# Rikorose/DeepFilterNet

Measured on NVIDIA H100. Metric: 48kHz audio-sec/sec (batched enhance), higher is better.
Workload: dtype f32 (bf16x3 tensor-core contractions, fp32 accumulate; DSP and gates IEEE fp32)

## Files before the change

### deepfilternet_b200/csrc/dfb_dwpw.cuh

```cuda
#pragma once
#include <cuda_runtime.h>
#include <stdint.h>

namespace dfb {

constexpr int kCh = 64;

__device__ __forceinline__ unsigned long long f2_pack(float lo, float hi) {
    unsigned long long r;
    asm("mov.b64 %0, {%1, %2};" : "=l"(r) : "f"(lo), "f"(hi));
    return r;
}
__device__ __forceinline__ void f2_unpack(unsigned long long v, float &lo, float &hi) {
    asm("mov.b64 {%0, %1}, %2;" : "=f"(lo), "=f"(hi) : "l"(v));
}
__device__ __forceinline__ unsigned long long f2_fma(unsigned long long a, unsigned long long b, unsigned long long c) {
    float a0, a1, b0, b1, c0, c1;
    f2_unpack(a, a0, a1);
    f2_unpack(b, b0, b1);
    f2_unpack(c, c0, c1);
    return f2_pack(fmaf(a0, b0, c0), fmaf(a1, b1, c1));
}

enum DwMode { DW_S1 = 0, DW_S2 = 1, DW_T2 = 2 };
constexpr int kLdA = kCh + 4;

struct DwPwParams {
    const float *in;
    const float *path;
    const float *ps, *pb;
    const float *dw;
    const float *pw;
    const float *bias;
    float *out;
    unsigned short *out_hi, *out_lo;
    int64_t in_fs, path_fs, out_fs;
    int T, Fin, Fout, kt, NF, lookahead;
    int fo_magic;
    const float *mk_e0;
    const float *mk_ps, *mk_pb;
    const float *mk_w;
    const float *mk_bias;
    float *mk_out;
    const int64_t *first;
    int64_t w0;
};


struct DwTaps {
    float4 wd[9];
    float4 ps4, pb4;
};

__device__ __forceinline__ void dw_load_taps(const DwPwParams &p, int cq, DwTaps &tp) {
#pragma unroll
    for (int i = 0; i < 9; i++) tp.wd[i] = make_float4(0.f, 0.f, 0.f, 0.f);
#pragma unroll
    for (int i = 0; i < 9; i++)
        if (i >= (3 - p.kt) * 3) tp.wd[i] = *reinterpret_cast<const float4 *>(p.dw + (i - (3 - p.kt) * 3) * kCh + cq * 4);
    tp.ps4 = make_float4(0.f, 0.f, 0.f, 0.f);
    tp.pb4 = tp.ps4;
    if (p.path) {
        tp.ps4 = *reinterpret_cast<const float4 *>(p.ps + cq * 4);
        tp.pb4 = *reinterpret_cast<const float4 *>(p.pb + cq * 4);
    }
}

template <int MODE>
__device__ __forceinline__ float4 dw_prologue(const DwPwParams &p, const DwTaps &tp, int b, int t, int fo, int cq) {
    float4 acc = make_float4(0.f, 0.f, 0.f, 0.f);
#pragma unroll
    for (int dt = 0; dt < 3; dt++) {
        if (dt < 3 - p.kt) continue;
        const int tq = t - (2 - dt) + p.lookahead;
        if (tq < 0 || tq >= p.T) continue;
#pragma unroll
        for (int df = 0; df < 3; df++) {
            int fi;
            float4 wv;
            if (MODE == DW_S1) { fi = fo + df - 1; wv = tp.wd[dt * 3 + df]; }
            else if (MODE == DW_S2) { fi = 2 * fo + df - 1; wv = tp.wd[dt * 3 + df]; }
            else {
                if (df == 2) continue;
                if ((fo & 1) == 0) { if (df == 1) continue; fi = fo >> 1; wv = tp.wd[dt * 3 + 1]; }
                else if (df == 0) { fi = fo >> 1; wv = tp.wd[dt * 3 + 2]; }
                else { fi = (fo >> 1) + 1; wv = tp.wd[dt * 3 + 0]; }
            }
            if (fi < 0 || fi >= p.Fin) continue;
            const int64_t o = ((int64_t)b * p.T + tq);
            float4 x = *reinterpret_cast<const float4 *>(p.in + o * p.in_fs + fi * kCh + cq * 4);
            if (p.path) {
                float4 e = *reinterpret_cast<const float4 *>(p.path + o * p.path_fs + fi * kCh + cq * 4);
                x.x += fmaxf(e.x * tp.ps4.x + tp.pb4.x, 0.f);
                x.y += fmaxf(e.y * tp.ps4.y + tp.pb4.y, 0.f);
                x.z += fmaxf(e.z * tp.ps4.z + tp.pb4.z, 0.f);
                x.w += fmaxf(e.w * tp.ps4.w + tp.pb4.w, 0.f);
            }
            acc.x += x.x * wv.x; acc.y += x.y * wv.y; acc.z += x.z * wv.z; acc.w += x.w * wv.w;
        }
// ... 6 lines not shown
```

### deepfilternet_b200/csrc/dfb_model.cu

```cuda
#include <cuda_bf16.h>

#include <algorithm>
#include <cmath>
#include <cstring>
#include <functional>
#include <map>
#include <numeric>
#include <string>

#include "dfb_common.cuh"
#include "dfb_dwpw.cuh"
#include "dfb_ptx.cuh"

namespace dfb {


enum Act { ACT_NONE = 0, ACT_RELU = 1, ACT_TANH = 2, ACT_SIGMOID = 3 };

__device__ __forceinline__ float act_apply(float x, int act) {
    switch (act) {
        case ACT_RELU: return fmaxf(x, 0.f);
        case ACT_TANH: return tanhf(x);
        case ACT_SIGMOID: return 1.f / (1.f + expf(-x));
        default: return x;
    }
}
__device__ __forceinline__ float sigmoidf_(float x) { return 1.f / (1.f + expf(-x)); }

constexpr int kInFrames = 8;
template <int CIN>
__global__ void __launch_bounds__(256)
k_conv_in(const float *__restrict__ x, const float *__restrict__ w , const float *__restrict__ bias,
          float *__restrict__ out, int T, int F, int kt, int lookahead, int Tsx ,
          int Tx ,
          int tp_min ,
          const RaggedRow *__restrict__ rg , int64_t w0 ,
          const int64_t *__restrict__ first ) {
    extern __shared__ float s_in[];
    const int b = blockIdx.y, t0 = blockIdx.x * kInFrames;
    const int rows = kInFrames + kt - 1, ld = (F + 2) * CIN;
    if (rg) Tx = min(Tx, (int)(rg[b].Tf - w0));
    if (first) tp_min = max(tp_min, stream_first(first, b, w0));
    for (int i = threadIdx.x; i < rows * ld; i += blockDim.x) {
        int r = i / ld, j = i - r * ld;
        int f = j / CIN - 1, ci = j - (f + 1) * CIN;
        int tp = t0 - (kt - 1) + r;
        float v = 0.f;
        if (f >= 0 && f < F && tp >= tp_min && tp + lookahead < Tx) v = x[(((int64_t)b * Tsx + tp + lookahead) * F + f) * CIN + ci];
        s_in[i] = v;
    }
    const int cq = threadIdx.x & 15, fl = threadIdx.x >> 4;
    unsigned long long wr[9 * CIN][2];
#pragma unroll
    for (int i = 0; i < 9 * CIN; i++) {
        const float4 v = (i >= (3 - kt) * 3 * CIN) ? *reinterpret_cast<const float4 *>(w + (i - (3 - kt) * 3 * CIN) * kCh + cq * 4)
                                                   : make_float4(0.f, 0.f, 0.f, 0.f);
        wr[i][0] = f2_pack(v.x, v.y); wr[i][1] = f2_pack(v.z, v.w);
    }
    const float4 bv = *reinterpret_cast<const float4 *>(bias + cq * 4);
    const unsigned long long b01 = f2_pack(bv.x, bv.y), b23 = f2_pack(bv.z, bv.w);
    __syncthreads();
    for (int fr = 0; fr < kInFrames; fr++) {
        int t = t0 + fr;
        if (t >= T) break;
        for (int f = fl; f < F; f += 16) {
            unsigned long long a01 = b01, a23 = b23;
#pragma unroll
            for (int dt = 0; dt < 3; dt++) {
                if (dt < 3 - kt) continue;
                const float *row = s_in + (fr + dt - (3 - kt)) * ld + f * CIN;
#pragma unroll
                for (int j = 0; j < 3 * CIN; j++) {
                    const float xv = row[j];
                    const unsigned long long xx = f2_pack(xv, xv);
                    a01 = f2_fma(xx, wr[dt * 3 * CIN + j][0], a01);
                    a23 = f2_fma(xx, wr[dt * 3 * CIN + j][1], a23);
                }
            }
            float4 acc;
            f2_unpack(a01, acc.x, acc.y); f2_unpack(a23, acc.z, acc.w);
            acc.x = fmaxf(acc.x, 0.f); acc.y = fmaxf(acc.y, 0.f); acc.z = fmaxf(acc.z, 0.f); acc.w = fmaxf(acc.w, 0.f);
            *reinterpret_cast<float4 *>(out + (((int64_t)b * T + t) * F + f) * kCh + cq * 4) = acc;
        }
    }
}

template <int MODE>
__global__ void __launch_bounds__(256) k_dwpw(DwPwParams p) {
    extern __shared__ __align__(16) float smem[];
    float *Ws = smem;
    float *As = smem + kCh * kCh;
    const int b = blockIdx.y, t0 = blockIdx.x * p.NF;
    const int tid = threadIdx.x;
    const int nf = min(p.NF, p.T - t0);
    const int R = nf * p.Fout;
// ... 587 lines not shown
extern "C" int64_t dfb_model_workspace_bytes(const dfb_model *m) { return m ? (int64_t)m->arena.cap : 0; }

namespace {

int run_gl(cudaStream_t s, const float *x, int64_t ldx, const float *w, const float *bias, const float *res,
           int64_t ldr, float *y, int64_t ldy, int64_t M, int G, int I, int Hh, int act, float oscale = 1.f,
           float ooffset = 0.f, unsigned short *y_hi = nullptr, unsigned short *y_lo = nullptr) {
    GlParams p{x, ldx, w, bias, res, ldr, y, ldy, M, G, I / G, Hh / G, act, oscale, ooffset, y_hi, y_lo};
    if ((p.Ig % 4) || (ldx % 4)) return fail(DFB_ERR_UNSUPPORTED, "grouped linear: K not a multiple of 4");
    if (G > 1 && (p.Hg % 4)) return fail(DFB_ERR_UNSUPPORTED, "grouped linear: group width %d not a multiple of 4", p.Hg);
    int tiles = (p.Hg + kGlBN - 1) / kGlBN;
    int gpc = (p.Hg < kGlBN && kGlBN % p.Hg == 0) ? (kGlBN / p.Hg < G ? kGlBN / p.Hg : G) : 1;
    dim3 grid((unsigned)((M + kGlBM - 1) / kGlBM), (unsigned)(((G + gpc - 1) / gpc) * tiles));
    static const bool detail = getenv("DFB_PROF_DETAIL") && atoi(getenv("DFB_PROF_DETAIL"));
    char name[64];
    if (detail) snprintf(name, sizeof name, "k_grouped_linear[%dx%d/%d]", I, Hh, G);
    else snprintf(name, sizeof name, "%s", p.G == 1 && p.bias && p.Hg >= 512 ? "k_grouped_linear[gru_proj]" : "k_grouped_linear");
    DFB_PROF(name, s);
    k_grouped_linear<<<grid, 256, 0, s>>>(p);
    DFB_LAUNCH_CHECK();
    return DFB_OK;
}

int run_gru(dfb_model *m, cudaStream_t s, const GruLayer *lw, int layers, int H, const float *res_last, float *y,
            float *xproj, int B, int T, const unsigned short *x_hi, const unsigned short *x_lo,
            unsigned short *pl_hi, unsigned short *pl_lo, int wide, unsigned short *out_hi, unsigned short *out_lo,
            bool *out_planes_ok, const GruChunk *ck) {
    if (out_planes_ok) *out_planes_ok = false;
    if (!x_hi || !x_lo || !pl_hi || !pl_lo) return fail(DFB_ERR_INVALID, "GRU: input planes and scratch planes are required");
    const int t0 = ck ? ck->t0 : 0, Tn = T - t0;
    const int64_t M = (int64_t)B * T;
    const unsigned short *cur_hi = x_hi, *cur_lo = x_lo;
    for (int l = 0; l < layers; l++) {
        const GruLayer &g = lw[l];
        int rc;
        if ((rc = launch_gemm_bf16x3(s, cur_hi, cur_lo, H, g.w_ih_hi, g.w_ih_lo, g.b_ih, xproj, 3 * H, M, 3 * H, H))) return rc;
        const bool last = l == layers - 1;
        float *dst = last ? y : nullptr;
        float *hs = ck && ck->h ? ck->h + (int64_t)l * ck->Bs * H : nullptr;
        GruWindow gw{ck && ck->have_state ? hs : nullptr, hs, t0, T, ck ? ck->first : nullptr, ck ? ck->w0 : 0};
        unsigned short *hi = last ? out_hi : pl_hi, *lo = last ? out_lo : pl_lo;
        if ((rc = launch_gru_tc(s, xproj, g.w_hh, g.b_hh, last ? res_last : nullptr, dst, hi, lo, B, Tn,
                                Tn <= m->gru_dbg_steps ? m->gru_dbg : nullptr, wide, last ? 1 : 0, &gw, H)))
            return rc;
        if (last && hi && out_planes_ok) *out_planes_ok = true;
        cur_hi = pl_hi; cur_lo = pl_lo;
    }
    return DFB_OK;
}

}
namespace dfb {
template <int MODE>
int launch_dwpw_tc(cudaStream_t s, DwPwParams p, const float *w_sw, int B);
}
namespace {

template <int MODE>
int run_dwpw(cudaStream_t s, DwPwParams p, int B, const float *w_sw = nullptr) {
    if (w_sw) return launch_dwpw_tc<MODE>(s, p, w_sw, B);
    static PerDeviceOnce attr_once;
    const int smem = (kCh * kCh + 128 * kLdA) * 4;
    if (auto once_guard = attr_once.first()) {
        DFB_CUDA(cudaFuncSetAttribute(k_dwpw<MODE>, cudaFuncAttributeMaxDynamicSharedMemorySize, smem));
    }
    p.NF = 128 / p.Fout;
    if (p.NF < 1) p.NF = 1;
    if (p.NF * p.Fout > 128 || (p.NF * p.Fout) % 4) return fail(DFB_ERR_UNSUPPORTED, "dwpw tile: Fout = %d", p.Fout);
    dim3 grid((unsigned)((p.T + p.NF - 1) / p.NF), (unsigned)B);
    DFB_PROF("k_dwpw", s);
    k_dwpw<MODE><<<grid, 256, smem, s>>>(p);
    DFB_LAUNCH_CHECK();
    return DFB_OK;
}

}

struct FwdBufs {
    float *e0, *e1, *e2, *e3, *c0, *c1, *emb_in, *emb, *g_a, *g_b, *xproj, *dec_emb, *d3, *d2, *d1, *dfc;
    unsigned short *ga_hi, *ga_lo, *gh_hi, *gh_lo;
    float *g_a2, *xproj2, *dfskip;
    unsigned short *ga2_hi, *ga2_lo, *gh2_hi, *gh2_lo;
    unsigned short *c1_hi, *c1_lo, *embin_hi, *embin_lo, *gb_hi, *gb_lo, *emb_hi, *emb_lo, *dfc_hi, *dfc_lo;
};

struct FwdBufsV1 {
    float *e0, *e1, *e2, *e3, *c0, *c1, *c1g, *cemb, *emb, *xproj, *xproj2, *y[3], *embo, *dec_old, *dec, *p3, *p2, *p1, *p0, *d3, *d2, *d1,
        *z[2], *dfc;
    unsigned short *emb_hi, *emb_lo, *y_hi[3], *y_lo[3], *embo_hi, *embo_lo, *z_hi[2], *z_lo[2], *dfc_hi, *dfc_lo, *scr_hi, *scr_lo;
};
static size_t fwd_plan_v1(const dfb_model_config &c, size_t M, Arena *a, FwdBufsV1 *f) {
    const int E = c.nb_erb, Fd = c.nb_df, H = c.emb_hidden;
    size_t bytes = 0;
    auto take = [&](size_t n) -> float * {
        bytes += (n * 4 + 255) & ~size_t(255);
        return a ? a->take<float>(n) : nullptr;
    };
    auto take16 = [&](size_t n) { return reinterpret_cast<unsigned short *>(take((n + 1) / 2)); };
    FwdBufsV1 t{};
    t.e0 = take(M * E * kCh); t.e1 = take(M * (E / 2) * kCh); t.e2 = take(M * (E / 4) * kCh); t.e3 = take(M * (E / 4) * kCh);
    t.c0 = take(M * Fd * kCh); t.c1 = take(M * (Fd / 2) * kCh); t.c1g = take(M * (Fd / 2) * kCh);
    t.cemb = take(M * H); t.emb = take(M * H); t.xproj = take(M * 3 * H); t.xproj2 = take(M * 3 * H);
    for (int i = 0; i < 3; i++) { t.y[i] = take(M * H); t.y_hi[i] = take16(M * H); t.y_lo[i] = take16(M * H); }
    for (int i = 0; i < 2; i++) { t.z[i] = take(M * H); t.z_hi[i] = take16(M * H); t.z_lo[i] = take16(M * H); }
    t.embo = take(M * H); t.dec_old = take(M * H); t.dec = take(M * H); t.dfc = take(M * H);
    t.p3 = take(M * (E / 4) * kCh); t.p2 = take(M * (E / 4) * kCh); t.p1 = take(M * (E / 2) * kCh); t.p0 = take(M * E * kCh);
    t.d3 = take(M * (E / 4) * kCh); t.d2 = take(M * (E / 2) * kCh); t.d1 = take(M * E * kCh);
    t.emb_hi = take16(M * H); t.emb_lo = take16(M * H); t.embo_hi = take16(M * H); t.embo_lo = take16(M * H);
    t.dfc_hi = take16(M * H); t.dfc_lo = take16(M * H); t.scr_hi = take16(M * H); t.scr_lo = take16(M * H);
    if (f) *f = t;
    return bytes + 4096;
}

// ... 128 lines not shown
    m->dbg["emb"] = {f.emb, M * emb_dim}; m->dbg["dec_emb"] = {f.dec_emb, M * ED}; m->dbg["d3"] = {f.d3, M * ED};
    m->dbg["d2"] = {f.d2, M * (E / 2) * kCh}; m->dbg["d1"] = {f.d1, M * E * kCh}; m->dbg["dfc"] = {f.dfc, M * Hd};
    m->dbg["g_a"] = {f.g_a, M * (H > Hd ? H : Hd)}; m->dbg["g_b"] = {f.g_b, M * (H > Hd ? H : Hd)};
    m->dbg["xproj"] = {f.xproj, M * 3 * (H > Hd ? H : Hd)};
    m->dbg["emb_in_hi"] = {reinterpret_cast<const float *>(f.embin_hi), M * emb_in_dim / 2};
    m->dbg["emb_in_lo"] = {reinterpret_cast<const float *>(f.embin_lo), M * emb_in_dim / 2};
    m->dbg["dfc_hi"] = {reinterpret_cast<const float *>(f.dfc_hi), M * Hd / 2};
    m->dbg["dfc_lo"] = {reinterpret_cast<const float *>(f.dfc_lo), M * Hd / 2};
    const int64_t e3_fs = c.enc_concat ? 2 * ED : ED;
    const bool keep_ga = c.model_kind == 2;
    float *const enc_ga = w.enc_in.bx ? nullptr : f.g_a;
    float *const erb_ga = !keep_ga && w.erb_in.bx ? nullptr : f.g_a;
    float *const df_ga = !keep_ga && w.df_in.bx ? nullptr : f.g_a2;
    float *const enc_gb = w.enc_out.bx ? nullptr : f.g_b;
    float *const erb_gb = w.erb_out.bx ? nullptr : f.g_b;
    float *const dfc = c.model_kind != 2 && w.df_out.bx ? nullptr : f.dfc;
    if (!erb_ga) m->dbg.erase("g_a");
    if (!erb_gb) m->dbg.erase("g_b");
    if (!dfc) m->dbg.erase("dfc");
    struct Pl { unsigned short *hi, *lo; int64_t ld; bool ok; };
    Pl pl_c1{f.c1_hi, f.c1_lo, (int64_t)Fd / 2 * kCh, false}, pl_embin{f.embin_hi, f.embin_lo, emb_in_dim, false},
       pl_gb{f.gb_hi, f.gb_lo, H, false}, pl_emb{f.emb_hi, f.emb_lo, emb_dim, false}, pl_dfc{f.dfc_hi, f.dfc_lo, Hd, false},
       pl_ga{f.ga_hi, f.ga_lo, H, false}, pl_ga2{f.ga2_hi, f.ga2_lo, Hd, false};
    auto ensure_planes = [&](cudaStream_t st, const float *x, int64_t ldx, int K, Pl &pl) -> int {
        if (pl.ok) return DFB_OK;
        if (pl.ld != K) return fail(DFB_ERR_INVALID, "plane pitch mismatch");
        if (!x) return fail(DFB_ERR_INVALID, "planes requested of an activation whose fp32 form was not written");
        int r = launch_to_planes(st, x, ldx, M, K, pl.hi, pl.lo);
        if (!r) pl.ok = true;
        return r;
    };
    auto gl = [&](cudaStream_t st, const Gl &g, const float *x, int64_t ldx, Pl *xin, int act,
                  const float *res, int64_t ldr, float *y, int64_t ldy, Pl *yout, int64_t ycol = 0) -> int {
        int r;
        unsigned short *yh = yout ? yout->hi + ycol : nullptr, *yl = yout ? yout->lo + ycol : nullptr;
        if (xin && g.bx) {
            if ((r = ensure_planes(st, x, ldx, g.I, *xin))) return r;
            r = launch_gl_bx(st, xin->hi, xin->lo, xin->ld, g.img, res, ldr, y, ldy, yh, yl, yout ? yout->ld : 0, M, g.G, g.I / g.G,
                             g.H / g.G, act, 1.f, 0.f);
            if (r != DFB_ERR_UNSUPPORTED) {
                if (!r && yout) yout->ok = true;
                return r;
            }
        }
        if (!x || !y)
            return fail(DFB_ERR_UNSUPPORTED, "grouped linear %dx%d/%d: the tensor-core kernel cannot take this launch and the fp32 %s "
                        "the FFMA kernel needs is not written", g.I, g.H, g.G, x ? "output" : "input");
        const bool ffma_planes = yout && yout->ld == ldy;
        r = run_gl(st, x, ldx, g.w, nullptr, res, ldr, y, ldy, M, g.G, g.I, g.H, act, 1.f, 0.f, ffma_planes ? yh : nullptr, ffma_planes ? yl : nullptr);
        if (!r && yout) yout->ok = ffma_planes;
        return r;
    };

    {
        dim3 grid((unsigned)((T + kInFrames - 1) / kInFrames), (unsigned)B);
        int smem = (kInFrames + c.inp_kt - 1) * (E + 2) * 4;
        DFB_PROF("k_conv_in[erb_conv0]", s);
        k_conv_in<1><<<grid, 256, smem, s>>>(d_feat_erb, w.erb_conv0.w, w.erb_conv0.b, f.e0, T, E, c.inp_kt, c.conv_lookahead, Tsx, Tx, 0, rows, W0, first);
        DFB_LAUNCH_CHECK();
    }
    cudaStream_t sa = serial ? s : L.aux;
    DFB_CUDA(cudaEventRecord(L.ev_fork_enc, s));
    DFB_CUDA(cudaStreamWaitEvent(sa, L.ev_fork_enc, 0));
    auto mk = [&](const Blk &k, const float *in, int Fin, int64_t in_fs, float *out, int Fout, int64_t out_fs, int kt) {
        DwPwParams p{};
        p.in = in; p.Fin = Fin; p.in_fs = in_fs; p.out = out; p.Fout = Fout; p.out_fs = out_fs; p.kt = kt; p.T = T;
        p.lookahead = 0;
        p.first = first; p.w0 = W0; p.dw = k.dw; p.bias = k.b;
        return p;
    };
    {
        {
            dim3 grid((unsigned)((T + kInFrames - 1) / kInFrames), (unsigned)B);
            int smem = (kInFrames + c.inp_kt - 1) * (Fd + 2) * 2 * 4;
            DFB_PROF("k_conv_in[df_conv0]", sa);
            k_conv_in<2><<<grid, 256, smem, sa>>>(d_feat_spec, w.df_conv0.w, w.df_conv0.b, f.c0, T, Fd, c.inp_kt, c.conv_lookahead, Tsx, Tx, 0, rows, W0, first);
            DFB_LAUNCH_CHECK();
            DFB_CUDA(cudaEventRecord(L.ev_c0, sa));
        }
        if (w.fused_emb) m->dbg.erase("c1");
        if (!w.fused_emb) {
            DwPwParams p = mk(w.df_conv1, f.c0, Fd, (int64_t)Fd * kCh, f.c1, Fd / 2, (int64_t)Fd / 2 * kCh, c.conv_kt);
            p.out_hi = pl_c1.hi; p.out_lo = pl_c1.lo; pl_c1.ok = true;
            if ((rc = run_dwpw<DW_S2>(sa, p, B, w.df_conv1.pw_sw))) return rc;
        }
        DFB_CUDA(cudaEventRecord(L.ev_join_enc, sa));
        DFB_CUDA(cudaStreamWaitEvent(sl, L.ev_c0, 0));
        if (!df_convp_built(c.df_order, c.df_pathway_kt))
            return fail(DFB_ERR_UNSUPPORTED, "df_order %d / df_pathway_kernel_size_t %d (built kernels: df_order 5, kt 1-5)",
                        c.df_order, c.df_pathway_kt);
        if (Fd % 2) return fail(DFB_ERR_UNSUPPORTED, "df pathway conv: odd nb_df");
        if ((rc = launch_df_convp_tc(sl, f.c0, w.df_convp.w_sw, w.df_convp.w2, w.df_convp.b, d_coefs, B, T, Fd, c.df_order,
                                     c.df_pathway_kt, first, W0)))
            return rc;
        DFB_CUDA(cudaEventRecord(L.ev_convp, sl));
    }
    {
        DwPwParams p = mk(w.erb_conv1, f.e0, E, (int64_t)E * kCh, f.e1, E / 2, (int64_t)E / 2 * kCh, c.conv_kt);
        if ((rc = run_dwpw<DW_S2>(s, p, B, w.erb_conv1.pw_sw))) return rc;
        p = mk(w.erb_conv2, f.e1, E / 2, (int64_t)E / 2 * kCh, f.e2, E / 4, (int64_t)E / 4 * kCh, c.conv_kt);
        if ((rc = run_dwpw<DW_S2>(s, p, B, w.erb_conv2.pw_sw))) return rc;
        p = mk(w.erb_conv3, f.e2, E / 4, (int64_t)E / 4 * kCh, f.e3, E / 4, e3_fs, c.conv_kt);
        if (c.enc_concat) { p.out_hi = pl_embin.hi; p.out_lo = pl_embin.lo; }
        if ((rc = run_dwpw<DW_S1>(s, p, B, w.erb_conv3.pw_sw))) return rc;

    }
    DFB_CUDA(cudaStreamWaitEvent(s, L.ev_join_enc, 0));
    {
        const int I = Fd / 2 * kCh;
        if (w.fused_emb) {
            const int G = c.g_df_fc_emb;
            rc = launch_df_emb(s, f.c0, M, T, Fd, c.conv_kt, w.df_conv1.dw, w.df_conv1.b, w.df_conv1.pw_sw, w.df_fc_emb.img, G, I / G, ED / G,
                               c.enc_concat ? nullptr : f.e3, ED, pl_embin.hi + (c.enc_concat ? ED : 0), pl_embin.lo + (c.enc_concat ? ED : 0),
                               pl_embin.ld, first, W0);
            if (!rc) pl_embin.ok = true;
            m->dbg.erase("emb_in");
        } else if (c.enc_concat) {
            rc = gl(s, w.df_fc_emb, f.c1, I, &pl_c1, ACT_RELU, nullptr, 0, f.emb_in + ED, emb_in_dim, &pl_embin, ED);
        } else {
            rc = gl(s, w.df_fc_emb, f.c1, I, &pl_c1, ACT_RELU, f.e3, ED, f.emb_in, emb_in_dim, &pl_embin);
        }
        if (rc) return rc;
    }
    {
        if ((rc = gl(s, w.enc_in, w.fused_emb ? nullptr : f.emb_in, emb_in_dim, &pl_embin, ACT_RELU, nullptr, 0, enc_ga, H, &pl_ga)))
            return rc;
        float *gout = c.g_enc_out ? enc_gb : f.emb;
        Pl &pl_gout = c.g_enc_out ? pl_gb : pl_emb;
        if ((rc = run_gru(m, s, w.enc_gru.data(), c.enc_gru_layers, H, nullptr, gout, f.xproj, B, T, f.ga_hi, f.ga_lo,
                          f.gh_hi, f.gh_lo, 0, pl_gout.hi, pl_gout.lo, &pl_gout.ok, cx ? &ck_enc : nullptr))) return rc;
        if (c.g_enc_out) {
            if ((rc = gl(s, w.enc_out, enc_gb, H, &pl_gb, ACT_RELU, nullptr, 0, f.emb, emb_dim, &pl_emb))) return rc;
        }
        if ((rc = ensure_planes(s, f.emb, emb_dim, emb_dim, pl_emb))) return rc;
        if (d_lsnr && (rc = run_gl(s, f.emb, emb_dim, w.lsnr.w, w.lsnr.b, nullptr, 0, d_lsnr, 1, M, 1, emb_dim, 1, ACT_SIGMOID, c.lsnr_scale,
                                   c.lsnr_offset)))
            return rc;
    }
    DFB_CUDA(cudaEventRecord(L.ev_fork, s));
    if (!serial) { s = L.dhi; sa = L.daux; DFB_CUDA(cudaStreamWaitEvent(s, L.ev_fork, 0)); }
    DFB_CUDA(cudaStreamWaitEvent(sa, L.ev_fork, 0));
    if (cx && cx->wait_dec) {
        DFB_CUDA(cudaStreamWaitEvent(s, cx->wait_dec, 0));
        DFB_CUDA(cudaStreamWaitEvent(sa, cx->wait_dec, 0));
    }
    static const char *wide_env = getenv("DFB_WIDE_BRANCH");
    const int wide_df = !wide_env || !strcmp(wide_env, "df") || !strcmp(wide_env, "both");
    const int wide_erb = wide_env && (!strcmp(wide_env, "erb") || !strcmp(wide_env, "both"));
    const bool early_skip = c.g_df_skip && c.model_kind != 2;
    if (early_skip) {
        if ((rc = gl(s, w.df_skip, f.emb, emb_dim, &pl_emb, ACT_NONE, nullptr, 0, f.dfskip, Hd, nullptr))) return rc;
        DFB_CUDA(cudaEventRecord(L.ev_skip, s));
// ... 2272 lines not shown
```

### deepfilternet_b200/csrc/dfb_tc.cu

```cuda
#include <cooperative_groups.h>
#include <atomic>
#include <map>
#include <mutex>
#include <cuda.h>
#include <cuda_bf16.h>

#include "dfb_common.cuh"
#include "dfb_dwpw.cuh"
#include "dfb_ptx.cuh"

namespace dfb {

constexpr int kBxBM = 128, kBxBN = 128, kBxBK = 64, kBxStages = 3, kBxThreads = 288;
constexpr int kBxBox = 128 * 128;

struct BxSmem {
    alignas(1024) unsigned char x[kBxStages][2][kBxBox];
    alignas(1024) unsigned char w[kBxStages][2][kBxBox];
    alignas(8) uint64_t full[kBxStages];
    uint64_t empty[kBxStages];
};

__global__ void __launch_bounds__(kBxThreads, 1)
k_gemm_bf16x3(const __grid_constant__ CUtensorMap tmXhi, const __grid_constant__ CUtensorMap tmXlo,
// ... 9 lines not shown
        fence_barrier_init();
    }
    __syncthreads();
    if (warp == 8) {
        if (lane == 0) {
            tma_prefetch_desc(&tmXhi); tma_prefetch_desc(&tmXlo); tma_prefetch_desc(&tmWhi); tma_prefetch_desc(&tmWlo);
            for (int kb = 0; kb < nkb; kb++) {
                const int s = kb % kBxStages, n = kb / kBxStages;
                if (n > 0) mbar_wait(&sm.empty[s], (n - 1) & 1);
                mbar_expect_tx(&sm.full[s], 4 * kBxBox);
                tma_load_2d(sm.x[s][0], &tmXhi, kb * kBxBK, m0, &sm.full[s]);
                tma_load_2d(sm.x[s][1], &tmXlo, kb * kBxBK, m0, &sm.full[s]);
                tma_load_2d(sm.w[s][0], &tmWhi, kb * kBxBK, n0, &sm.full[s]);
                tma_load_2d(sm.w[s][1], &tmWlo, kb * kBxBK, n0, &sm.full[s]);
            }
        }
        return;
    }
    const int wm = (warp & 3) * 32, wn = (warp >> 2) * 64;
    float acc[2][8][4];
#pragma unroll
    for (int a = 0; a < 2; a++)
#pragma unroll
        for (int b = 0; b < 8; b++)
#pragma unroll
            for (int c = 0; c < 4; c++) acc[a][b][c] = 0.f;
    for (int kb = 0; kb < nkb; kb++) {
        const int s = kb % kBxStages;
        mbar_wait(&sm.full[s], (kb / kBxStages) & 1);
        warp_mma_sw128_k64<2>(smem_u32(sm.x[s][0]), smem_u32(sm.x[s][1]), smem_u32(sm.w[s][0]), smem_u32(sm.w[s][1]), wm, wn, acc);
        __syncwarp();
        if (lane == 0) mbar_arrive(&sm.empty[s]);
    }
#pragma unroll
    for (int nt = 0; nt < 8; nt++) {
        const int n = n0 + wn + 8 * nt + 2 * (lane & 3);
        const float2 bn = bias ? make_float2(__ldg(bias + n), __ldg(bias + n + 1)) : make_float2(0.f, 0.f);
#pragma unroll
        for (int mt = 0; mt < 2; mt++)
#pragma unroll
            for (int h = 0; h < 2; h++) {
                const int m = m0 + wm + 16 * mt + (lane >> 2) + 8 * h;
                if (m < M)
                    *reinterpret_cast<float2 *>(Y + (int64_t)m * ldy + n) =
                        make_float2(acc[mt][nt][2 * h] + bn.x, acc[mt][nt][2 * h + 1] + bn.y);
            }
    }
}

constexpr int kDxThreads = 256;
constexpr uint32_t kDxW = 32768, kDxRaw = 49152, kDxTail = 64 * 4 + 32;


template <int MODE, int KT, int PATH, int MASK>
__global__ void __launch_bounds__(kDxThreads, 2)
k_dwpw_bx(DwPwParams p, const float *__restrict__ w_sw ) {
    extern __shared__ __align__(1024) unsigned char tc_smem_raw[];
    const uint32_t sb = smem_u32(tc_smem_raw);
    if (sb & 1023u) __trap();
    const int tid = threadIdx.x, warp = tid >> 5, lane = tid & 31;
    const int b = blockIdx.y, t0 = blockIdx.x * p.NF;
    const int nf = min(p.NF, p.T - t0);
    const int R = nf * p.Fout;
    const int tq0 = t0 - (KT - 1);
    const uint32_t fbytes = (uint32_t)p.Fin * kCh * 4;
    const uint32_t raw_in = sb + kDxRaw, raw_path = raw_in + (uint32_t)(p.NF + KT - 1) * fbytes;
    const uint32_t raw_e0 = raw_in + (uint32_t)(p.NF + KT - 1) * fbytes * (PATH ? 2u : 1u);
    const uint32_t obytes = (uint32_t)p.Fout * kCh * 4;
    const uint32_t tail = raw_e0 + (MASK ? (uint32_t)p.NF * obytes : 0u);
    const uint32_t s_bias = tail, bar_raw = tail + 264;
    const uint32_t s_mask = raw_in;
    if (tid == 0) {
        mbar_init_a(bar_raw, 1);
        fence_barrier_init();
        const int ta = max(tq0, 0), tb = t0 + nf;
        mbar_expect_tx_a(bar_raw, (uint32_t)(tb - ta) * fbytes * (PATH ? 2u : 1u) + 2u * kCh * 128u + (MASK ? (uint32_t)nf * obytes : 0u));
        if (MASK)
            for (int t = t0; t < tb; t++)
                bulk_load(raw_e0 + (uint32_t)(t - t0) * obytes, p.mk_e0 + ((int64_t)b * p.T + t) * p.Fout * kCh, obytes, bar_raw);
        for (int t = ta; t < tb; t++) {
            bulk_load(raw_in + (uint32_t)(t - tq0) * fbytes, p.in + ((int64_t)b * p.T + t) * p.in_fs, fbytes, bar_raw);
            if (PATH) bulk_load(raw_path + (uint32_t)(t - tq0) * fbytes, p.path + ((int64_t)b * p.T + t) * p.path_fs, fbytes, bar_raw);
        }
        bulk_load(sb + kDxW, w_sw, 2 * kCh * 128, bar_raw);
    }
    if (tid < kCh / 4) sts128(s_bias + tid * 16, __ldg(reinterpret_cast<const float4 *>(p.bias) + tid));
    const int cq = tid & 15, slot = tid >> 4;
    float4 wd[KT][3], ps4, pb4;
#pragma unroll
    for (int dt = 0; dt < KT; dt++)
#pragma unroll
        for (int df = 0; df < 3; df++) wd[dt][df] = __ldg(reinterpret_cast<const float4 *>(p.dw + (dt * 3 + df) * kCh) + cq);
    if (PATH) {
        ps4 = __ldg(reinterpret_cast<const float4 *>(p.ps) + cq);
        pb4 = __ldg(reinterpret_cast<const float4 *>(p.pb) + cq);
    }
    int fr = (8 * slot * p.fo_magic) >> 16, fo = 8 * slot - fr * p.Fout;
    __syncthreads();
    mbar_wait_a(bar_raw, 0);
    auto rd = [&](uint32_t a) -> float4 {
        float4 x = lds128(a);
        if (PATH) {
            const float4 e = lds128(a + (raw_path - raw_in));
            x.x += fmaxf(fmaf(e.x, ps4.x, pb4.x), 0.f); x.y += fmaxf(fmaf(e.y, ps4.y, pb4.y), 0.f);
            x.z += fmaxf(fmaf(e.z, ps4.z, pb4.z), 0.f); x.w += fmaxf(fmaf(e.w, ps4.w, pb4.w), 0.f);
        }
        return x;
    };
    const float4 zero4 = make_float4(0.f, 0.f, 0.f, 0.f);
    const int t_first = KT > 1 ? stream_first(p.first, b, p.w0) : 0;
#pragma unroll
    for (int i = 0; i < 8; i++) {
        const int r = 8 * slot + i;
        float4 acc = zero4;
        if (r < R) {
#pragma unroll
            for (int dt = 0; dt < KT; dt++) {
                if (KT > 1 && tq0 + fr + dt < t_first) continue;
                const uint32_t fb = raw_in + (uint32_t)(fr + dt) * fbytes + cq * 16;
                if (MODE == DW_S1) {
                    const uint32_t a = fb + (uint32_t)fo * 256;
                    if (fo > 0) acc = f4_fma(rd(a - 256), wd[dt][0], acc);
                    acc = f4_fma(rd(a), wd[dt][1], acc);
                    if (fo + 1 < p.Fin) acc = f4_fma(rd(a + 256), wd[dt][2], acc);
                } else if (MODE == DW_S2) {
                    const uint32_t a = fb + (uint32_t)fo * 512;
                    if (fo > 0) acc = f4_fma(rd(a - 256), wd[dt][0], acc);
                    acc = f4_fma(rd(a), wd[dt][1], acc);
                    acc = f4_fma(rd(a + 256), wd[dt][2], acc);
                } else {
                    const uint32_t a = fb + (uint32_t)(fo >> 1) * 256;
                    if ((fo & 1) == 0) {
                        acc = f4_fma(rd(a), wd[dt][1], acc);
                    } else {
                        acc = f4_fma(rd(a), wd[dt][2], acc);
                        if ((fo >> 1) + 1 < p.Fin) acc = f4_fma(rd(a + 256), wd[dt][0], acc);
                    }
                }
            }
        }
// ... 47 lines not shown
                const int f2 = f0 + i, r2 = r0 + i;
                if (f2 < 0 || f2 >= p.Fout) continue;
                const float4 d = lds128(sb + r2 * 256 + ((j ^ (r2 & 15)) << 4));
                const float4 e = lds128(raw_e0 + r2 * 256 + j * 16);
                float4 x;
                x.x = fmaxf(fmaf(e.x, s4.x, b4.x), 0.f) + d.x; x.y = fmaxf(fmaf(e.y, s4.y, b4.y), 0.f) + d.y;
                x.z = fmaxf(fmaf(e.z, s4.z, b4.z), 0.f) + d.z; x.w = fmaxf(fmaf(e.w, s4.w, b4.w), 0.f) + d.w;
                if (i + 1 < 8) part[i + 1 < 0 ? 0 : i + 1] += x.x * w0.x + x.y * w0.y + x.z * w0.z + x.w * w0.w;
                if (i >= 0 && i < 8) part[i < 0 ? 0 : (i > 7 ? 7 : i)] += x.x * w1.x + x.y * w1.y + x.z * w1.z + x.w * w1.w;
                if (i - 1 >= 0) part[i - 1 > 7 ? 7 : i - 1] += x.x * w2.x + x.y * w2.y + x.z * w2.z + x.w * w2.w;
            }
        }
#pragma unroll
        for (int i = 0; i < 8; i++) {
            float v = part[i];
            v += __shfl_xor_sync(0xffffffffu, v, 1);
            v += __shfl_xor_sync(0xffffffffu, v, 2);
            v += __shfl_xor_sync(0xffffffffu, v, 4);
            v += __shfl_xor_sync(0xffffffffu, v, 8);
            part[i] = v;
        }
        if (r0 < R && j < 8) {
            float z = part[0];
#pragma unroll
            for (int i = 1; i < 8; i++) z = j == i ? part[i] : z;
            z += __ldg(p.mk_bias);
            p.mk_out[((int64_t)b * p.T + t0 + fr) * p.Fout + f0 + j] = 1.f / (1.f + expf(-z));
        }
    }
    if (p.out || p.out_hi) {
        const int j = tid & 15;
        int fr2 = (8 * slot * p.fo_magic) >> 16, fo2 = 8 * slot - fr2 * p.Fout;
        int64_t off = ((int64_t)b * p.T + t0 + fr2) * p.out_fs + fo2 * kCh + j * 4;
#pragma unroll
        for (int i = 0; i < 8; i++) {
            const int r = 8 * slot + i;
            if (r < R) {
                const float4 v = lds128(sb + r * 256 + ((j ^ (r & 15)) << 4));
                if (p.out) *reinterpret_cast<float4 *>(p.out + off) = v;
                if (p.out_hi) {
                    uint32_t h0, l0, h1, l1;
                    bf16x2_split(v.x, v.y, h0, l0);
                    bf16x2_split(v.z, v.w, h1, l1);
                    *reinterpret_cast<uint2 *>(p.out_hi + off) = make_uint2(h0, h1);
                    *reinterpret_cast<uint2 *>(p.out_lo + off) = make_uint2(l0, l1);
                }
            }
            off += kCh;
            if (++fo2 == p.Fout) { fo2 = 0; off += p.out_fs - (int64_t)p.Fout * kCh; }
        }
    }
}

template <int MODE, int KT, int PATH, int MASK = 0>
static int launch_dwpw_bx(cudaStream_t s, const DwPwParams &p, const float *w_sw, int B) {
    static int attr_smem[64] = {0};
    int dev = 0;
    cudaGetDevice(&dev);
    dev &= 63;
    const int raw = (p.NF + KT - 1) * p.Fin * kCh * 4 * (PATH ? 2 : 1) + (MASK ? p.NF * p.Fout * kCh * 4 : 0);
    const int smem = (int)kDxRaw + raw + (int)kDxTail;
    if (smem > 227 * 1024) return fail(DFB_ERR_UNSUPPORTED, "dwpw tile needs %d bytes of shared memory", smem);
    if (smem > attr_smem[dev]) {
        DFB_CUDA(cudaFuncSetAttribute(k_dwpw_bx<MODE, KT, PATH, MASK>, cudaFuncAttributeMaxDynamicSharedMemorySize, smem));
        attr_smem[dev] = smem;
    }
    dim3 grid((unsigned)((p.T + p.NF - 1) / p.NF), (unsigned)B);
    DFB_PROF("k_dwpw_bx", s);
    k_dwpw_bx<MODE, KT, PATH, MASK><<<grid, kDxThreads, smem, s>>>(p, w_sw);
    DFB_LAUNCH_CHECK();
    return DFB_OK;
}

template <int MODE>
int launch_dwpw_tc(cudaStream_t s, DwPwParams p, const float *w_sw, int B) {
    p.NF = 128 / p.Fout;
    if (p.NF < 1) p.NF = 1;
    if (p.NF * p.Fout > 128) return fail(DFB_ERR_UNSUPPORTED, "dwpw tile: Fout = %d", p.Fout);
    p.fo_magic = (65536 + p.Fout - 1) / p.Fout;
    for (int r = 0; r < 128; r++)
        if (((r * p.fo_magic) >> 16) != r / p.Fout) return fail(DFB_ERR_UNSUPPORTED, "dwpw tile: Fout = %d", p.Fout);
    if ((p.in_fs * 4) % 16 || (p.path && (p.path_fs * 4) % 16)) return fail(DFB_ERR_UNSUPPORTED, "dwpw: unaligned frame stride");
    const bool path = p.path != nullptr;
    if (MODE == DW_S1) {
        if (p.kt == 1) return path ? launch_dwpw_bx<DW_S1, 1, 1>(s, p, w_sw, B) : launch_dwpw_bx<DW_S1, 1, 0>(s, p, w_sw, B);
        if (p.kt == 2) return path ? launch_dwpw_bx<DW_S1, 2, 1>(s, p, w_sw, B) : launch_dwpw_bx<DW_S1, 2, 0>(s, p, w_sw, B);
    } else if (MODE == DW_S2 && !path) {
        if (p.kt == 1) return launch_dwpw_bx<DW_S2, 1, 0>(s, p, w_sw, B);
        if (p.kt == 2) return launch_dwpw_bx<DW_S2, 2, 0>(s, p, w_sw, B);
    } else if (MODE == DW_T2 && path && p.kt == 1) {
        if (p.mk_e0) {
            return launch_dwpw_bx<DW_T2, 1, 1, 1>(s, p, w_sw, B);
        }
        return launch_dwpw_bx<DW_T2, 1, 1>(s, p, w_sw, B);
    }
    return fail(DFB_ERR_UNSUPPORTED, "dwpw tensor-core path: mode %d kt %d path %d", MODE, p.kt, (int)path);
}
template int launch_dwpw_tc<DW_S1>(cudaStream_t, DwPwParams, const float *, int);
template int launch_dwpw_tc<DW_S2>(cudaStream_t, DwPwParams, const float *, int);
template int launch_dwpw_tc<DW_T2>(cudaStream_t, DwPwParams, const float *, int);

constexpr int kCvThreads = 256, kCvOut = 124, kCvYld = 51 , kCvBins = 8;
constexpr uint32_t kCvW = 32768, kCvRawOff = 49152, kCvYs = kCvRawOff + 32768, kCvTail = kCvYs + 128 * kCvYld * 4;

struct CvParams {
    const float *w_sw;
    const float *w2;
    const float *bias;
    float *coefs;
    int T, Fd;
    const int64_t *first;
    int64_t w0;
};

template <int ORDER, int KTP>
__global__ void __launch_bounds__(kCvThreads, 2) k_df_convp_tc(const __grid_constant__ CUtensorMap tmC0, CvParams p) {
    constexpr int O2 = 2 * ORDER, NY = KTP * ORDER;
    extern __shared__ __align__(1024) unsigned char tc_smem_raw[];
    const uint32_t sb = (smem_u32(tc_smem_raw) + 1023u) & ~1023u;
    const int tid = threadIdx.x, warp = tid >> 5, lane = tid & 31;
    const int f_begin = blockIdx.x * kCvBins, f_end = min(f_begin + kCvBins, p.Fd);
    const int b = blockIdx.z, t0 = blockIdx.y * kCvOut, r0 = t0 - (KTP - 1);
    const uint32_t s_w2 = sb + kCvTail, bar_raw = s_w2 + 512, bar_w = bar_raw + 16;
    const int row = b * p.T + r0;
    auto load_bin = [&](int f) {
        mbar_expect_tx_a(bar_raw, 32768);
        asm volatile("cp.async.bulk.tensor.2d.shared::cluster.global.mbarrier::complete_tx::bytes [%0], [%1, {%2, %3}], [%4];"
                     ::"r"(sb + kCvRawOff), "l"((uint64_t)&tmC0), "r"(f * 64), "r"(row), "r"(bar_raw) : "memory");
        asm volatile("cp.async.bulk.tensor.2d.shared::cluster.global.mbarrier::complete_tx::bytes [%0], [%1, {%2, %3}], [%4];"
                     ::"r"(sb + kCvRawOff + 16384), "l"((uint64_t)&tmC0), "r"(f * 64 + 32), "r"(row), "r"(bar_raw) : "memory");
    };
    if (tid == 0) {
        mbar_init_a(bar_raw, 1);
        mbar_init_a(bar_w, 1);
        fence_barrier_init();
        mbar_expect_tx_a(bar_w, 16384);
        bulk_load(sb + kCvW, p.w_sw, 16384, bar_w);
        load_bin(f_begin);
    }
    for (int i = tid; i < O2 * O2 + O2; i += kCvThreads)
        asm volatile("st.shared.f32 [%0], %1;" ::"r"(s_w2 + 4 * i), "f"(i < O2 * O2 ? __ldg(p.w2 + i) : __ldg(p.bias + i - O2 * O2)) : "memory");
    __syncthreads();
    mbar_wait_a(bar_w, 0);
    const int r = tid & 127, half = tid >> 7;
    const bool zero = r0 + r < stream_first(p.first, b, p.w0);
    for (int f = f_begin, it = 0; f < f_end; f++, it++) {
        const uint32_t par = (uint32_t)(it & 1);
        mbar_wait_a(bar_raw, par);
        {
            const uint32_t src = sb + kCvRawOff + (uint32_t)half * 16384u + (uint32_t)r * 128u;
            float4 xs[8];
#pragma unroll
            for (int c = 0; c < 8; c++) xs[c] = lds128(src + (uint32_t)((c ^ (r & 7)) << 4));
// ... 507 lines not shown
```

Measured before the change: 71650.

## Fuse ERB input conv0 into the first stride-2 depthwise/pointwise tensor-core kernel

Measured after the change: 71870 (median of 6 runs). About the same (+0.3%).

```diff
diff --git a/deepfilternet_b200/csrc/dfb_dwpw.cuh b/deepfilternet_b200/csrc/dfb_dwpw.cuh
--- a/deepfilternet_b200/csrc/dfb_dwpw.cuh
+++ b/deepfilternet_b200/csrc/dfb_dwpw.cuh
@@ -1,6 +1,8 @@
 #pragma once
 #include <cuda_runtime.h>
 #include <stdint.h>
+
+#include "dfb_common.cuh"
 
 namespace dfb {
 
@@ -25,6 +27,13 @@
 enum DwMode { DW_S1 = 0, DW_S2 = 1, DW_T2 = 2 };
 constexpr int kLdA = kCh + 4;
 
+struct ErbIn {
+    const float *x, *w, *b;
+    float *e0;
+    const RaggedRow *rows;
+    int Tsx, Tx, lookahead, kt;
+};
+
 struct DwPwParams {
     const float *in;
     const float *path;
@@ -45,6 +54,50 @@
     const int64_t *first;
     int64_t w0;
 };
+
+
+__device__ __forceinline__ void conv_in_bounds(const RaggedRow *rg, const int64_t *first, int b, int64_t w0, int &tp_min, int &Tx) {
+    if (rg) Tx = min(Tx, (int)(rg[b].Tf - w0));
+    if (first) tp_min = max(tp_min, stream_first(first, b, w0));
+}
+
+__device__ __forceinline__ void erb_conv0_stage(float *s_in, const float *__restrict__ x, int b, int tp0, int rows, int F, int lookahead,
+                                                int Tsx, int tp_min, int Tx, int i0, int stride) {
+    const int ld = F + 2;
+    for (int i = i0; i < rows * ld; i += stride) {
+        int r = i / ld, f = i - r * ld - 1;
+        int tp = tp0 + r;
+        float v = 0.f;
+        if (f >= 0 && f < F && tp >= tp_min && tp + lookahead < Tx) v = x[((int64_t)b * Tsx + tp + lookahead) * F + f];
+        s_in[i] = v;
+    }
+}
+
+__device__ __forceinline__ void erb_conv0_taps(const float *__restrict__ w, const float *__restrict__ bias, int kt, int cq,
+                                               float4 (&wq)[9], float4 &bq) {
+#pragma unroll
+    for (int i = 0; i < 9; i++)
+        wq[i] = (i >= (3 - kt) * 3) ? *reinterpret_cast<const float4 *>(w + (i - (3 - kt) * 3) * kCh + cq * 4)
+                                    : make_float4(0.f, 0.f, 0.f, 0.f);
+    bq = *reinterpret_cast<const float4 *>(bias + cq * 4);
+}
+
+__device__ __forceinline__ float4 erb_conv0_quad(const float *s, int ld, int kt, const float4 (&wq)[9], float4 acc) {
+#pragma unroll
+    for (int dt = 0; dt < 3; dt++) {
+        if (dt < 3 - kt) continue;
+        const float *row = s + (dt - (3 - kt)) * ld;
+#pragma unroll
+        for (int j = 0; j < 3; j++) {
+            const float xv = row[j];
+            const float4 wv = wq[dt * 3 + j];
+            acc.x = fmaf(xv, wv.x, acc.x); acc.y = fmaf(xv, wv.y, acc.y);
+            acc.z = fmaf(xv, wv.z, acc.z); acc.w = fmaf(xv, wv.w, acc.w);
+        }
+    }
+    acc.x = fmaxf(acc.x, 0.f); acc.y = fmaxf(acc.y, 0.f); acc.z = fmaxf(acc.z, 0.f); acc.w = fmaxf(acc.w, 0.f);
+    return acc;
+}
 
 
 struct DwTaps {
diff --git a/deepfilternet_b200/csrc/dfb_model.cu b/deepfilternet_b200/csrc/dfb_model.cu
--- a/deepfilternet_b200/csrc/dfb_model.cu
+++ b/deepfilternet_b200/csrc/dfb_model.cu
@@ -39,8 +39,21 @@
     extern __shared__ float s_in[];
     const int b = blockIdx.y, t0 = blockIdx.x * kInFrames;
     const int rows = kInFrames + kt - 1, ld = (F + 2) * CIN;
-    if (rg) Tx = min(Tx, (int)(rg[b].Tf - w0));
-    if (first) tp_min = max(tp_min, stream_first(first, b, w0));
+    conv_in_bounds(rg, first, b, w0, tp_min, Tx);
+    if constexpr (CIN == 1) {
+        const int cq = threadIdx.x & 15, fl = threadIdx.x >> 4;
+        erb_conv0_stage(s_in, x, b, t0 - (kt - 1), rows, F, lookahead, Tsx, tp_min, Tx, threadIdx.x, blockDim.x);
+        float4 wq[9], bq;
+        erb_conv0_taps(w, bias, kt, cq, wq, bq);
+        __syncthreads();
+        for (int fr = 0; fr < kInFrames; fr++) {
+            int t = t0 + fr;
+            if (t >= T) break;
+            for (int f = fl; f < F; f += 16)
+                *reinterpret_cast<float4 *>(out + (((int64_t)b * T + t) * F + f) * kCh + cq * 4) = erb_conv0_quad(s_in + fr * ld + f, ld, kt, wq, bq);
+        }
+        return;
+    }
     for (int i = threadIdx.x; i < rows * ld; i += blockDim.x) {
         int r = i / ld, j = i - r * ld;
         int f = j / CIN - 1, ci = j - (f + 1) * CIN;
@@ -734,13 +747,13 @@
 }
 namespace dfb {
 template <int MODE>
-int launch_dwpw_tc(cudaStream_t s, DwPwParams p, const float *w_sw, int B);
+int launch_dwpw_tc(cudaStream_t s, DwPwParams p, const float *w_sw, int B, const ErbIn &x0c);
 }
 namespace {
 
 template <int MODE>
-int run_dwpw(cudaStream_t s, DwPwParams p, int B, const float *w_sw = nullptr) {
-    if (w_sw) return launch_dwpw_tc<MODE>(s, p, w_sw, B);
+int run_dwpw(cudaStream_t s, DwPwParams p, int B, const float *w_sw = nullptr, const ErbIn &x0c = ErbIn{}) {
+    if (w_sw) return launch_dwpw_tc<MODE>(s, p, w_sw, B, x0c);
     static PerDeviceOnce attr_once;
     const int smem = (kCh * kCh + 128 * kLdA) * 4;
     if (auto once_guard = attr_once.first()) {
@@ -975,13 +988,6 @@
         return r;
     };
 
-    {
-        dim3 grid((unsigned)((T + kInFrames - 1) / kInFrames), (unsigned)B);
-        int smem = (kInFrames + c.inp_kt - 1) * (E + 2) * 4;
-        DFB_PROF("k_conv_in[erb_conv0]", s);
-        k_conv_in<1><<<grid, 256, smem, s>>>(d_feat_erb, w.erb_conv0.w, w.erb_conv0.b, f.e0, T, E, c.inp_kt, c.conv_lookahead, Tsx, Tx, 0, rows, W0, first);
-        DFB_LAUNCH_CHECK();
-    }
     cudaStream_t sa = serial ? s : L.aux;
     DFB_CUDA(cudaEventRecord(L.ev_fork_enc, s));
     DFB_CUDA(cudaStreamWaitEvent(sa, L.ev_fork_enc, 0));
@@ -1019,8 +1025,9 @@
         DFB_CUDA(cudaEventRecord(L.ev_convp, sl));
     }
     {
-        DwPwParams p = mk(w.erb_conv1, f.e0, E, (int64_t)E * kCh, f.e1, E / 2, (int64_t)E / 2 * kCh, c.conv_kt);
-        if ((rc = run_dwpw<DW_S2>(s, p, B, w.erb_conv1.pw_sw))) return rc;
+        DwPwParams p = mk(w.erb_conv1, nullptr, E, (int64_t)E * kCh, f.e1, E / 2, (int64_t)E / 2 * kCh, c.conv_kt);
+        const ErbIn x0c{d_feat_erb, w.erb_conv0.w, w.erb_conv0.b, f.e0, rows, Tsx, Tx, c.conv_lookahead, c.inp_kt};
+        if ((rc = run_dwpw<DW_S2>(s, p, B, w.erb_conv1.pw_sw, x0c))) return rc;
         p = mk(w.erb_conv2, f.e1, E / 2, (int64_t)E / 2 * kCh, f.e2, E / 4, (int64_t)E / 4 * kCh, c.conv_kt);
         if ((rc = run_dwpw<DW_S2>(s, p, B, w.erb_conv2.pw_sw))) return rc;
         p = mk(w.erb_conv3, f.e2, E / 4, (int64_t)E / 4 * kCh, f.e3, E / 4, e3_fs, c.conv_kt);
diff --git a/deepfilternet_b200/csrc/dfb_tc.cu b/deepfilternet_b200/csrc/dfb_tc.cu
--- a/deepfilternet_b200/csrc/dfb_tc.cu
+++ b/deepfilternet_b200/csrc/dfb_tc.cu
@@ -85,9 +85,9 @@
 constexpr uint32_t kDxW = 32768, kDxRaw = 49152, kDxTail = 64 * 4 + 32;
 
 
-template <int MODE, int KT, int PATH, int MASK>
+template <int MODE, int KT, int PATH, int MASK, int IN0>
 __global__ void __launch_bounds__(kDxThreads, 2)
-k_dwpw_bx(DwPwParams p, const float *__restrict__ w_sw ) {
+k_dwpw_bx(DwPwParams p, const float *__restrict__ w_sw , ErbIn x0c) {
     extern __shared__ __align__(1024) unsigned char tc_smem_raw[];
     const uint32_t sb = smem_u32(tc_smem_raw);
     if (sb & 1023u) __trap();
@@ -107,18 +107,37 @@
         mbar_init_a(bar_raw, 1);
         fence_barrier_init();
         const int ta = max(tq0, 0), tb = t0 + nf;
-        mbar_expect_tx_a(bar_raw, (uint32_t)(tb - ta) * fbytes * (PATH ? 2u : 1u) + 2u * kCh * 128u + (MASK ? (uint32_t)nf * obytes : 0u));
+        mbar_expect_tx_a(bar_raw, (IN0 ? 0u : (uint32_t)(tb - ta) * fbytes * (PATH ? 2u : 1u)) + 2u * kCh * 128u + (MASK ? (uint32_t)nf * obytes : 0u));
         if (MASK)
             for (int t = t0; t < tb; t++)
                 bulk_load(raw_e0 + (uint32_t)(t - t0) * obytes, p.mk_e0 + ((int64_t)b * p.T + t) * p.Fout * kCh, obytes, bar_raw);
-        for (int t = ta; t < tb; t++) {
-            bulk_load(raw_in + (uint32_t)(t - tq0) * fbytes, p.in + ((int64_t)b * p.T + t) * p.in_fs, fbytes, bar_raw);
-            if (PATH) bulk_load(raw_path + (uint32_t)(t - tq0) * fbytes, p.path + ((int64_t)b * p.T + t) * p.path_fs, fbytes, bar_raw);
-        }
+        if (!IN0)
+            for (int t = ta; t < tb; t++) {
+                bulk_load(raw_in + (uint32_t)(t - tq0) * fbytes, p.in + ((int64_t)b * p.T + t) * p.in_fs, fbytes, bar_raw);
+                if (PATH) bulk_load(raw_path + (uint32_t)(t - tq0) * fbytes, p.path + ((int64_t)b * p.T + t) * p.path_fs, fbytes, bar_raw);
+            }
         bulk_load(sb + kDxW, w_sw, 2 * kCh * 128, bar_raw);
     }
     if (tid < kCh / 4) sts128(s_bias + tid * 16, __ldg(reinterpret_cast<const float4 *>(p.bias) + tid));
     const int cq = tid & 15, slot = tid >> 4;
+    if constexpr (IN0) {
+        const int E = p.Fin, ld = E + 2;
+        const int ta = max(tq0, 0), tb = t0 + nf;
+        float *xs = reinterpret_cast<float *>(tc_smem_raw);
+        int tp_min = 0, Tx = x0c.Tx;
+        conv_in_bounds(x0c.rows, p.first, b, p.w0, tp_min, Tx);
+        erb_conv0_stage(xs, x0c.x, b, ta - (x0c.kt - 1), tb - ta + x0c.kt - 1, E, x0c.lookahead, x0c.Tsx, tp_min, Tx, tid, kDxThreads);
+        float4 wq[9], bq;
+        erb_conv0_taps(x0c.w, x0c.b, x0c.kt, cq, wq, bq);
+        __syncthreads();
+        for (int t = ta; t < tb; t++)
+            for (int f = slot; f < E; f += 16) {
+                const float4 e = erb_conv0_quad(xs + (t - ta) * ld + f, ld, x0c.kt, wq, bq);
+                sts128(raw_in + (uint32_t)(t - tq0) * fbytes + (uint32_t)f * 256 + cq * 16, e);
+                if (t >= t0)
+                    *reinterpret_cast<float4 *>(x0c.e0 + (((int64_t)b * p.T + t) * E + f) * kCh + cq * 4) = e;
+            }
+    }
     float4 wd[KT][3], ps4, pb4;
 #pragma unroll
     for (int dt = 0; dt < KT; dt++)
@@ -272,8 +291,8 @@
     }
 }
 
-template <int MODE, int KT, int PATH, int MASK = 0>
-static int launch_dwpw_bx(cudaStream_t s, const DwPwParams &p, const float *w_sw, int B) {
+template <int MODE, int KT, int PATH, int MASK = 0, int IN0 = 0>
+static int launch_dwpw_bx(cudaStream_t s, const DwPwParams &p, const float *w_sw, int B, const ErbIn &x0c) {
     static int attr_smem[64] = {0};
     int dev = 0;
     cudaGetDevice(&dev);
@@ -282,18 +301,18 @@
     const int smem = (int)kDxRaw + raw + (int)kDxTail;
     if (smem > 227 * 1024) return fail(DFB_ERR_UNSUPPORTED, "dwpw tile needs %d bytes of shared memory", smem);
     if (smem > attr_smem[dev]) {
-        DFB_CUDA(cudaFuncSetAttribute(k_dwpw_bx<MODE, KT, PATH, MASK>, cudaFuncAttributeMaxDynamicSharedMemorySize, smem));
+        DFB_CUDA(cudaFuncSetAttribute(k_dwpw_bx<MODE, KT, PATH, MASK, IN0>, cudaFuncAttributeMaxDynamicSharedMemorySize, smem));
         attr_smem[dev] = smem;
     }
     dim3 grid((unsigned)((p.T + p.NF - 1) / p.NF), (unsigned)B);
     DFB_PROF("k_dwpw_bx", s);
-    k_dwpw_bx<MODE, KT, PATH, MASK><<<grid, kDxThreads, smem, s>>>(p, w_sw);
+    k_dwpw_bx<MODE, KT, PATH, MASK, IN0><<<grid, kDxThreads, smem, s>>>(p, w_sw, x0c);
     DFB_LAUNCH_CHECK();
     return DFB_OK;
 }
 
 template <int MODE>
-int launch_dwpw_tc(cudaStream_t s, DwPwParams p, const float *w_sw, int B) {
+int launch_dwpw_tc(cudaStream_t s, DwPwParams p, const float *w_sw, int B, const ErbIn &x0c) {
     p.NF = 128 / p.Fout;
     if (p.NF < 1) p.NF = 1;
     if (p.NF * p.Fout > 128) return fail(DFB_ERR_UNSUPPORTED, "dwpw tile: Fout = %d", p.Fout);
@@ -303,22 +322,25 @@
     if ((p.in_fs * 4) % 16 || (p.path && (p.path_fs * 4) % 16)) return fail(DFB_ERR_UNSUPPORTED, "dwpw: unaligned frame stride");
     const bool path = p.path != nullptr;
     if (MODE == DW_S1) {
-        if (p.kt == 1) return path ? launch_dwpw_bx<DW_S1, 1, 1>(s, p, w_sw, B) : launch_dwpw_bx<DW_S1, 1, 0>(s, p, w_sw, B);
-        if (p.kt == 2) return path ? launch_dwpw_bx<DW_S1, 2, 1>(s, p, w_sw, B) : launch_dwpw_bx<DW_S1, 2, 0>(s, p, w_sw, B);
+        if (p.kt == 1) return path ? launch_dwpw_bx<DW_S1, 1, 1>(s, p, w_sw, B, x0c) : launch_dwpw_bx<DW_S1, 1, 0>(s, p, w_sw, B, x0c);
+        if (p.kt == 2) return path ? launch_dwpw_bx<DW_S1, 2, 1>(s, p, w_sw, B, x0c) : launch_dwpw_bx<DW_S1, 2, 0>(s, p, w_sw, B, x0c);
+    } else if (MODE == DW_S2 && !path && x0c.x) {
+        if (p.kt == 1) return launch_dwpw_bx<DW_S2, 1, 0, 0, 1>(s, p, w_sw, B, x0c);
+        if (p.kt == 2) return launch_dwpw_bx<DW_S2, 2, 0, 0, 1>(s, p, w_sw, B, x0c);
     } else if (MODE == DW_S2 && !path) {
-        if (p.kt == 1) return launch_dwpw_bx<DW_S2, 1, 0>(s, p, w_sw, B);
-        if (p.kt == 2) return launch_dwpw_bx<DW_S2, 2, 0>(s, p, w_sw, B);
+        if (p.kt == 1) return launch_dwpw_bx<DW_S2, 1, 0>(s, p, w_sw, B, x0c);
+        if (p.kt == 2) return launch_dwpw_bx<DW_S2, 2, 0>(s, p, w_sw, B, x0c);
     } else if (MODE == DW_T2 && path && p.kt == 1) {
         if (p.mk_e0) {
-            return launch_dwpw_bx<DW_T2, 1, 1, 1>(s, p, w_sw, B);
-        }
-        return launch_dwpw_bx<DW_T2, 1, 1>(s, p, w_sw, B);
+            return launch_dwpw_bx<DW_T2, 1, 1, 1>(s, p, w_sw, B, x0c);
+        }
+        return launch_dwpw_bx<DW_T2, 1, 1>(s, p, w_sw, B, x0c);
     }
     return fail(DFB_ERR_UNSUPPORTED, "dwpw tensor-core path: mode %d kt %d path %d", MODE, p.kt, (int)path);
 }
-template int launch_dwpw_tc<DW_S1>(cudaStream_t, DwPwParams, const float *, int);
-template int launch_dwpw_tc<DW_S2>(cudaStream_t, DwPwParams, const float *, int);
-template int launch_dwpw_tc<DW_T2>(cudaStream_t, DwPwParams, const float *, int);
+template int launch_dwpw_tc<DW_S1>(cudaStream_t, DwPwParams, const float *, int, const ErbIn &);
+template int launch_dwpw_tc<DW_S2>(cudaStream_t, DwPwParams, const float *, int, const ErbIn &);
+template int launch_dwpw_tc<DW_T2>(cudaStream_t, DwPwParams, const float *, int, const ErbIn &);
 
 constexpr int kCvThreads = 256, kCvOut = 124, kCvYld = 51 , kCvBins = 8;
 constexpr uint32_t kCvW = 32768, kCvRawOff = 49152, kCvYs = kCvRawOff + 32768, kCvTail = kCvYs + 128 * kCvYld * 4;
```
